# AlvinHon/ring-zk

Measured on AMD Instinct MI355X. Metric: proofs/sec (commit+challenge+response+verify), N=1024, batch=4096; NTT GB/s vs HBM peak, higher is better.
Workload: dtype u32

## Files before the change

ring_zk_amd/csrc/rzk_rowprog.h:

```cpp
#pragma once
#include "rzk_wave.h"

namespace rzk {

__device__ __forceinline__ int32_t canon_lo(int64_t c, uint32_t qhalf, uint32_t& bad) {
  bad |= (uint32_t)(((uint64_t)c + qhalf) >> 32);
  return (int32_t)c;
}
__device__ __forceinline__ int32_t canon_lo_mx(int64_t c, uint32_t qhalf, uint32_t& bad, uint32_t& mx) {
  const uint64_t s = (uint64_t)c + qhalf;
  bad |= (uint32_t)(s >> 32);
  const uint32_t lo = (uint32_t)s;
  mx = lo > mx ? lo : mx;
  return (int32_t)c;
}
__device__ __forceinline__ void canon_pair(const longlong2 t, uint32_t qhalf, uint32_t& bad, uint32_t& mx, int32_t& lo0,
                                           int32_t& lo1) {
  lo0 = canon_lo_mx(t.x, qhalf, bad, mx);
  lo1 = canon_lo_mx(t.y, qhalf, bad, mx);
}
__device__ __forceinline__ bool canon_fail(uint32_t bad, uint32_t mx, uint32_t qhalf) {
  return __any((bad != 0) | (mx > 2u * qhalf)) != 0;
}
__device__ __forceinline__ void input_fault(const Operands& ops, uint8_t* flags, uint32_t bo, int lane) {
// ... 279 lines not shown
    suma += a[i] < 0 ? 0u - ua : ua;
  }
  const double bound = (double)TM::sum_u56(suma) * (double)TM::max_u32(maxv);
  const int npass = __builtin_amdgcn_readfirstlane(bound < 4.0e18 ? 1 : 2);
  int32_t* list = ext + S::WORDS;
  uint32_t lbase = 0, ltotal = 1;
  if (LIST) {
    const uint32_t mine = shift_count_nonzeros<E>(a);
    const uint32_t w = (uint32_t)__builtin_amdgcn_readfirstlane(lane >> 6);
    if ((lane & 63) == 0) list[2 * kShiftListCap + w] = (int32_t)mine;
    TM::sync();
    const uint32_t c0 = (uint32_t)__builtin_amdgcn_readfirstlane(list[2 * kShiftListCap]);
    const uint32_t c1 = (uint32_t)__builtin_amdgcn_readfirstlane(list[2 * kShiftListCap + 1]);
    lbase = w ? c0 : 0u;
    ltotal = c0 + c1;
  }
  bool started = false;
#pragma unroll 1
  for (int pass = 0; pass < npass; ++pass) {
    if (npass == 2) {
      uint32_t u0 = 0, u1 = 0, u2 = 0;
      TM::sync();
      shift_fill_from<LOGN, PAIR, LL>(pv, lane, ext, pass == 0 ? SHIFT_LOW16 : SHIFT_HIGH16, false, false, qhalf, u0, u1, u2);
    }
    if (!LIST || npass == 2) TM::sync();
#pragma unroll 1
    for (uint32_t r0 = 0; r0 < (ltotal ? ltotal : 1u); r0 += LIST ? (uint32_t)kShiftListCap : 1u) {
      uint32_t nent = 0;
      if (LIST) {
        if (r0 || pass) TM::sync();
        shift_list_write<LOGN, PAIR, LL>(a, lane, lbase, r0, list);
        TM::sync();
        nent = ltotal - r0 < (uint32_t)kShiftListCap ? ltotal - r0 : (uint32_t)kShiftListCap;
      }
#pragma unroll 1
      for (int ch = 0; ch < NCH; ++ch) {
        int64_t acc[H];
#pragma unroll
        for (int i = 0; i < H; ++i) acc[i] = 0;
        if (LIST) shift_scan_list<LOGN, PAIR, LL, H>(acc, list, nent, lane, ext + ch * (S::LANES * H));
        else shift_scan<LOGN, PAIR, H>(acc, a, lane, ext + ch * (S::LANES * H));
#pragma unroll
        for (int i = 0; i < H; ++i) {
          uint32_t u = zq_from_i64(acc[i], T.crt);
          if (pass) u = montq_u(u, T.crt.r48q, T.crt);
          if (TO_MEM) {
            uint32_t* slot = res + S::j(lane, i) + ch * (S::LANES * H);
            const uint32_t cur = (fresh && !started) ? 0u : *slot;
            *slot = minus ? subq(cur, u, q) : addq(cur, u, q);
          } else {
#pragma unroll
            for (int c = 0; c < NCH; ++c) {
              const uint32_t cur = res[c * H + i];
              const uint32_t nw = minus ? subq(cur, u, q) : addq(cur, u, q);
              res[c * H + i] = c == ch ? nw : cur;
            }
          }
        }
      }
      started = true;
    }
  }
}

template <int LOGN>
__device__ __forceinline__ bool shift_product_bytes(uint32_t* res, bool minus, const int32_t* a, const int64_t* __restrict__ pv,
                                                    int lane, int32_t* slab, const DevTables& T, bool& fault, bool trusted) {
  using S = ShiftGeo<LOGN, true>;
  using B = ByteGeo<LOGN>;
  constexpr int E = S::E;
  const uint32_t q = T.crt.q, qhalf = T.crt.qhalf;
  uint32_t* img = reinterpret_cast<uint32_t*>(slab);
  uint32_t vbad = 0, vmx = 0, maxv = 0, suma = 0;
#pragma unroll
  for (int i = 0; i < E; ++i) {
    const uint32_t ua = (uint32_t)a[i], aa = a[i] < 0 ? 0u - ua : ua;
    suma += aa < 256u ? aa : 256u;
  }
  const uint32_t norm1 = wave_sum_u32(suma);
  if (norm1 > 255u) return false;
  wave_sync();
  constexpr int GH = S::G / 2;
  const longlong2* __restrict__ p = reinterpret_cast<const longlong2*>(pv) + lane;
#pragma unroll 1
  for (int h = 0; h < 2; ++h) {
    int32_t vh[2 * GH];
#pragma unroll
    for (int g = 0; g < GH; ++g) {
      const longlong2 t = ld_stream(p + (h * GH + g) * 64);
      if (trusted) vh[2 * g] = (int32_t)t.x, vh[2 * g + 1] = (int32_t)t.y;
      else canon_pair(t, qhalf, vbad, vmx, vh[2 * g], vh[2 * g + 1]);
    }
#pragma unroll
    for (int g = 0; g < GH; ++g) {
#pragma unroll
      for (int c = 0; c < 2; ++c) {
        const uint32_t uv = (uint32_t)vh[2 * g + c], av = vh[2 * g + c] < 0 ? 0u - uv : uv;
        maxv = av > maxv ? av : maxv;
      }
      shift_bytes_put_raw<LOGN>(vh[2 * g], vh[2 * g + 1], lane, h * GH + g, img);
    }
    if (h == 0 && wave_max_u32(maxv) > 127u) return false;
  }
  const uint32_t bias = wave_max_u32(maxv);
  if (!shift_bytes_ok(norm1, bias)) return false;
  if (!trusted) fault = fault || canon_fail(vbad, vmx, qhalf);
  wave_sync();
  shift_bytes_bias<LOGN>(lane, bias, img);
  wave_sync();
  uint32_t acc[B::W];
#pragma unroll
  for (int k = 0; k < B::W; ++k) acc[k] = 0;
#pragma unroll
  for (int i = 0; i < E; ++i) {
    uint64_t mask = __ballot(a[i] != 0);
    while (mask) {
      const int l = __builtin_ctzll(mask);
      mask &= mask - 1;
      const int32_t coef = __builtin_amdgcn_readlane(a[i], l);
      int ln = lane;
      asm volatile("" : "+v"(ln));
      shift_bytes_accum<LOGN>(acc, ln, S::off(i) + 2 * l, coef, img);
    }
  }
  wave_sync();
  shift_bytes_park<LOGN>(acc, lane, img);
  wave_sync();
  int32_t prod[E];
  shift_bytes_take<LOGN>(prod, lane, norm1 * bias, img);
#pragma unroll
  for (int i = 0; i < E; ++i) {
    const uint32_t u = zq_from_centered(prod[i], q);
    res[i] = minus ? subq(res[i], u, q) : addq(res[i], u, q);
  }
  return true;
}

template <int LOGN, class TM>
__device__ __forceinline__ void store_operand_image(const uint32_t* x, const Operands& ops, uint32_t op, uint32_t off, uint32_t b,
                                                    int pi, int lane, float nrm2, bool first) {
  using G = Geo<LOGN, TM::LL>;
  if (!ops.oimg || op != ops.oimg_op || off >= 32u) return;
  const int ci = ops.oimg_col[off];
  if (ci < 0) return;
  const size_t oslot = (size_t)b * ops.oimg_n + (uint32_t)ci;
  uint4* __restrict__ dst = reinterpret_cast<uint4*>(ops.oimg + (oslot * kKeyImages + pi) * G::N);
#pragma unroll
  for (int g = 0; g < G::E / 4; ++g) dst[G::key4(lane, g)] = make_uint4(x[4 * g], x[4 * g + 1], x[4 * g + 2], x[4 * g + 3]);
  if (lane == 0) {
    if (first) ops.oimg_l2[oslot] = (double)nrm2;
    ops.oimg_np[oslot] = (uint8_t)(pi + 1);
  }
}

template <int LOGN, bool HAS_VEC, bool OPQ = false, class TM = WaveTeam, bool DD = false>
__device__ __forceinline__ void term_direct(uint32_t* acc, const Term tm, const Operands& ops, uint32_t b,
                                            uint32_t bo, int lane, uint32_t* lds, const uint32_t* __restrict__ twf,
                                            const PrimeConsts& pc, int pi, const uint32_t* __restrict__ key_ntt,
                                            const double* __restrict__ key_l2, bool first, float& bound,
                                            uint8_t* __restrict__ flags, uint32_t qhalf) {
  using G = Geo<LOGN, TM::LL>;
  constexpr int E = G::E;
  constexpr int N = G::N;
  int ln = lane;
  RZK_OPAQUE(ln);
  uint32_t x[E];
  float nb = 0.f;
  bool below = true, fault = false;
  const bool chk = first && (tm.kind & (TERM_CHECK | TERM_CHECK2));
  const bool trusted = ops.trusted != 0;
  bool from_image = false;
  size_t oslot = 0;
  if (DD && (tm.kind & TERM_KIND_MASK) == TERM_DD && ops.oimg) {
    const uint32_t summand = tm.b_off / ops.oimg_k, col = tm.b_off - summand * ops.oimg_k;
    const int ci = col < 32u ? ops.oimg_col[col] : -1;
    if (ci >= 0) {
      oslot = ((size_t)bo * ops.oimg_group + summand) * ops.oimg_n + (uint32_t)ci;
      from_image = (int)ops.oimg_np[oslot] > pi;
    }
  }
  if (DD) from_image = __builtin_amdgcn_readfirstlane((int)from_image) != 0;
  if (DD && from_image) {
    const uint4* __restrict__ ip = reinterpret_cast<const uint4*>(ops.oimg + (oslot * kKeyImages + pi) * N);
#pragma unroll
    for (int g = 0; g < E / 4; ++g) {
      const uint4 iv = ip[G::key4(ln, g)];
      x[4 * g] = iv.x, x[4 * g + 1] = iv.y, x[4 * g + 2] = iv.z, x[4 * g + 3] = iv.w;
    }
    nb = (float)ops.oimg_l2[oslot];
  } else {
    load_lift<LOGN, TM, kRowLoadMode<TM>>(x, operand_ptr(ops, tm.b_op, tm.b_off, b, bo, N), ln, pc, first, nb, chk, ops.norm_limit, below, qhalf, trusted, fault);
    if (chk && !below && (lane & 63) == 0) fail_check(flags + bo, ops.pad != 0, (tm.kind & TERM_CHECK2) != 0);
    wave_fwd<LOGN, TM>(x, ln, lds, twf, pc);
  }
  if (HAS_VEC && (tm.kind & TERM_KIND_MASK) == TERM_VEC) {
    uint32_t xb[E];
#pragma unroll
    for (int c = 0; c < E; ++c) xb[c] = csub(mont_lazy(x[c], pc.ninv_r2, pc.p, pc.npinv), pc.p);
    float na = 0.f;
    bool unused_below = true;
    load_lift<LOGN, TM, kRowLoadMode<TM>>(x, operand_ptr(ops, tm.a_op, tm.a_off, b, bo, N), ln, pc, first, na, false, 0, unused_below, qhalf, trusted, fault);
    wave_fwd<LOGN, TM>(x, ln, lds, twf, pc);
    if (first) bound = bound_fma(na, nb, bound);
    if (tm.sign >= 0) {
#pragma unroll
      for (int c = 0; c < E; ++c) acc[c] = mac_add(acc[c], x[c], xb[c], pc);
    } else {
#pragma unroll
      for (int c = 0; c < E; ++c) acc[c] = mac_sub(acc[c], x[c], xb[c], pc);
    }
  } else {
    const bool dk = (tm.kind & TERM_KIND_MASK) == TERM_DKEY || (tm.kind & TERM_KIND_MASK) == TERM_DD;
    const size_t image = dk ? (size_t)bo * ops.dkey_n + tm.a_off : (size_t)tm.a_off;
    if (first) bound = bound_fma((float)(dk ? ops.dkey_l2[image] : key_l2[image]), nb, bound);
    const uint4* __restrict__ kp = reinterpret_cast<const uint4*>((dk ? ops.dkey_img : key_ntt) + (image * kKeyImages + pi) * N);
    if (tm.sign >= 0) {
#pragma unroll
      for (int g = 0; g < E / 4; ++g) {
        const uint4 kv = kp[G::key4(ln, g)];
        acc[4 * g + 0] = mac_add(acc[4 * g + 0], x[4 * g + 0], kv.x, pc);
        acc[4 * g + 1] = mac_add(acc[4 * g + 1], x[4 * g + 1], kv.y, pc);
        acc[4 * g + 2] = mac_add(acc[4 * g + 2], x[4 * g + 2], kv.z, pc);
        acc[4 * g + 3] = mac_add(acc[4 * g + 3], x[4 * g + 3], kv.w, pc);
      }
    } else {
#pragma unroll
      for (int g = 0; g < E / 4; ++g) {
        const uint4 kv = kp[G::key4(ln, g)];
        acc[4 * g + 0] = mac_sub(acc[4 * g + 0], x[4 * g + 0], kv.x, pc);
        acc[4 * g + 1] = mac_sub(acc[4 * g + 1], x[4 * g + 1], kv.y, pc);
        acc[4 * g + 2] = mac_sub(acc[4 * g + 2], x[4 * g + 2], kv.z, pc);
        acc[4 * g + 3] = mac_sub(acc[4 * g + 3], x[4 * g + 3], kv.w, pc);
      }
    }
  }
  if (fault) input_fault(ops, flags, bo, lane);
}

template <int LOGN, bool OPQ = false, class TM = WaveTeam>
__device__ __forceinline__ void inverse_and_fold(int pi, int np, uint32_t* acc, int lane, uint32_t* lds,
                                                 const uint32_t* __restrict__ twi, const PrimeConsts& pc,
                                                 uint32_t* st_lds, uint32_t* __restrict__ st_glb, const DevTables& T) {
  using G = Geo<LOGN, TM::LL>;
  constexpr int E = G::E;
  int li = lane;
  RZK_OPAQUE(li);
  wave_inv<LOGN, TM>(acc, li, lds, twi, pc);
  if (pi == 0) {
#pragma unroll
    for (int e = 0; e < E; ++e) st_lds[G::j_p1(li, e)] = crt_fold0(acc[e], np, T.pc, T.crt);
  } else if (pi == 1) {
    uint32_t d0[E];
#pragma unroll
    for (int e = 0; e < E; ++e) {
      d0[e] = st_lds[G::j_p1(li, e)];
      acc[e] = crt_digit1(acc[e], d0[e], np, T.pc, T.crt);
    }
    if (np == 3) {
#pragma unroll
      for (int e = 0; e < E; ++e) st_glb[G::j_p1(li, e)] = crt_value01_modp2(d0[e], acc[e], T.pc, T.crt);
    }
#pragma unroll
    for (int e = 0; e < E; ++e) st_lds[G::j_p1(li, e)] = crt_value01_modq(d0[e], acc[e], T.crt);
  } else {
#pragma unroll
    for (int e = 0; e < E; ++e) {
      uint32_t a = st_lds[G::j_p1(li, e)];
      crt_fold2(acc[e], T.pc, T.crt, a, st_glb[G::j_p1(li, e)]);
      st_lds[G::j_p1(li, e)] = a;
    }
  }
}

template <int LOGN, class TM = WaveTeam>
__device__ __forceinline__ void checked_add_verdicts(const Program* __restrict__ prog, const Row row, const Operands& ops,
                                                     uint32_t b, uint32_t bo, int lane, const float* add_ss,
                                                     uint8_t* __restrict__ flags) {
  using G = Geo<LOGN, TM::LL>;
#pragma unroll 1
  for (uint32_t a = 0; a < row.nadds && a < 4; ++a) {
    const AddTerm ad = table_load(&prog->adds[row.add0 + a]);
    if (!(ad.op & (ADD_CHECK | ADD_CHECK2))) continue;
    float part = 0.f;
#pragma unroll
    for (int sl = 0; sl < 4; ++sl) part = (sl == (int)a) ? add_ss[sl] : part;
    const double sfl = (double)TM::sum_f32(part), lim = (double)ops.norm_limit;
    bool below;
    if (sfl * (1.0 + 2.0 * (double)kNormSlack) < lim) {
      below = true;
    } else if (sfl * (1.0 - 2.0 * (double)kNormSlack) >= lim) {
      below = false;
    } else {
      const int64_t* __restrict__ src = operand_ptr(ops, ad.op & ADD_OP_MASK, ad.off, b, bo, G::N);
      int32_t v[G::E];
#pragma unroll
      for (int e = 0; e < G::E; ++e) v[e] = (int32_t)src[G::j_p1(lane, e)];
      below = TM::sum_u56(lane_sum_sq_exact<G::E>(v)) < ops.norm_limit;
    }
    if (!below && (lane & 63) == 0) fail_check(flags + bo, ops.pad != 0, (ad.op & ADD_CHECK2) != 0);
  }
}

template <int LOGN, int CH, class TM = WaveTeam>
__device__ __forceinline__ void add_chunk(uint32_t* u, const AddTerm ad, uint32_t a, const int64_t* __restrict__ src, int lane,
                                          int e0, uint32_t q, uint32_t qhalf, bool trusted, uint32_t& in_bad, uint32_t& in_mx,
                                          float* add_ss) {
  using G = Geo<LOGN, TM::LL>;
  int32_t av[CH];
  if (trusted) {
#pragma unroll
    for (int i = 0; i < CH; ++i) av[i] = (int32_t)ld_stream(src + G::j_p1(lane, e0 + i));
  } else {
#pragma unroll
    for (int i = 0; i < CH; ++i) av[i] = canon_lo_mx(ld_stream(src + G::j_p1(lane, e0 + i)), qhalf, in_bad, in_mx);
  }
  if (ad.op & (ADD_CHECK | ADD_CHECK2)) {
    float sq = 0.f;
#pragma unroll
    for (int i = 0; i < CH; ++i) {
      const float f = (float)av[i];
      sq = __builtin_fmaf(f, f, sq);
    }
    const uint32_t slot = a < 4 ? a : 3;
#pragma unroll
    for (int sl = 0; sl < 4; ++sl) add_ss[sl] += (sl == (int)slot) ? sq : 0.f;
  }
  if (ad.sign >= 0) {
#pragma unroll
    for (int i = 0; i < CH; ++i) u[i] = addq(u[i], zq_from_centered(av[i], q), q);
  } else {
#pragma unroll
    for (int i = 0; i < CH; ++i) u[i] = subq(u[i], zq_from_centered(av[i], q), q);
  }
}

template <int LOGN, class TM = WaveTeam>
__device__ __forceinline__ void row_epilogue(const Program* __restrict__ prog, const Row row, const Operands& ops,
                                             uint32_t b, uint32_t bo, int lane, bool has_terms, int np,
                                             const uint32_t* st_lds, const DevTables& T, uint8_t* __restrict__ flags,
                                             const uint32_t* __restrict__ st_sh = nullptr) {
  using G = Geo<LOGN, TM::LL>;
  constexpr int E = G::E;
  constexpr int N = G::N;
  int nz = 0;
  constexpr int CH = kEpiChunk < E ? kEpiChunk : E;
  const uint32_t q = T.crt.q;
  const bool trusted = ops.trusted != 0;
  float add_ss[4] = {0.f, 0.f, 0.f, 0.f};
  uint32_t in_bad = 0, in_mx = 0;
#pragma unroll
  for (int e0 = 0; e0 < E; e0 += CH) {
    uint32_t u[CH];
    if (has_terms) {
#pragma unroll
      for (int i = 0; i < CH; ++i) u[i] = crt_finish_zq(st_lds[G::j_p1(lane, e0 + i)], np, T.crt);
    } else {
#pragma unroll
      for (int i = 0; i < CH; ++i) u[i] = 0;
    }
    if (st_sh) {
#pragma unroll
      for (int i = 0; i < CH; ++i) u[i] = addq(u[i], st_sh[G::j_p1(lane, e0 + i)], q);
    }
#pragma unroll 1
    for (uint32_t a = 0; a < row.nadds; ++a) {
      const AddTerm ad = table_load(&prog->adds[row.add0 + a]);
      add_chunk<LOGN, CH, TM>(u, ad, a, operand_ptr(ops, ad.op & ADD_OP_MASK, ad.off, b, bo, N), lane, e0, q, T.crt.qhalf, trusted,
                          in_bad, in_mx, add_ss);
    }
    if (row.mode == MODE_STORE) {
      int64_t* __restrict__ dst = const_cast<int64_t*>(operand_ptr(ops, row.out_op, row.out_off, b, bo, N));
#pragma unroll
      for (int i = 0; i < CH; ++i) st_stream(dst + G::j_p1(lane, e0 + i), center_from_zq(u[i], T.crt));
    } else {
#pragma unroll
      for (int i = 0; i < CH; ++i) nz |= (u[i] != 0);
    }
  }
  if (row.mode != MODE_STORE) {
    if (__any(nz) && (lane & 63) == 0) flags[bo] = 0;
  }
  if (row.nadds && !trusted && canon_fail(in_bad, in_mx, T.crt.qhalf)) input_fault(ops, flags, bo, lane);
  if (ops.norm_limit) checked_add_verdicts<LOGN, TM>(prog, row, ops, b, bo, lane, add_ss, flags);
}

__device__ __forceinline__ int primes_for(float fbound, const DevTables& T) {
  const double bound = (double)fbound * (1.0 + 0x1p-12);
  const int np = bound <= T.cap[1] ? 1 : (bound <= T.cap[2] ? 2 : 3);
  return __builtin_amdgcn_readfirstlane(np);
}

}
```

ring_zk_amd/csrc/rzk_unit.h:

```cpp
#pragma once
#include "rzk_rowprog.h"

namespace rzk {

constexpr int kScratchLines = 6;
#ifndef RZK_STAMPS
#define RZK_STAMPS 0
#endif
#if RZK_STAMPS
#define RZK_T0() const uint64_t t_sec0 = __builtin_amdgcn_s_memtime()
#define RZK_T1(acc) acc += __builtin_amdgcn_s_memtime() - t_sec0
#else
#define RZK_T0() do { } while (0)
#define RZK_T1(acc) do { } while (0)
#endif

__device__ __forceinline__ void set_priority_level(uint32_t level) {
  if (level == 0) __builtin_amdgcn_s_setprio(3);
  else if (level == 1) __builtin_amdgcn_s_setprio(2);
  else if (level == 2) __builtin_amdgcn_s_setprio(1);
  else __builtin_amdgcn_s_setprio(0);
}
__device__ __forceinline__ void set_progress_priority(uint32_t done, uint32_t total) {
  set_priority_level(__builtin_amdgcn_readfirstlane(total ? (done * 4u) / total : 0u));
}
template <int LOGN, bool to_regs, bool MINUS, class TM = WaveTeam>
__device__ __forceinline__ void mac_park_signed(uint32_t* x, const uint32_t* mul, uint4* P4, int lane, bool init,
                                                const PrimeConsts& pc) {
  using G = Geo<LOGN, TM::LL>;
  constexpr int E = G::E;
  if (init && !MINUS) {
#pragma unroll
    for (int g = 0; g < E / 4; ++g) {
      uint32_t as[4];
#pragma unroll
      for (int i = 0; i < 4; ++i) as[i] = mont_lazy(x[4 * g + i], mul[4 * g + i], pc.p, pc.npinv);
      if (to_regs) {
#pragma unroll
        for (int i = 0; i < 4; ++i) x[4 * g + i] = as[i];
      } else {
        P4[G::own4(lane, g)] = make_uint4(as[0], as[1], as[2], as[3]);
      }
    }
    return;
  }
#pragma unroll
  for (int g = 0; g < E / 4; ++g) {
    uint4 a = make_uint4(0, 0, 0, 0);
    if (!init) a = P4[G::own4(lane, g)];
    uint32_t as[4] = {a.x, a.y, a.z, a.w};
#pragma unroll
    for (int i = 0; i < 4; ++i)
      as[i] = MINUS ? mac_sub(as[i], x[4 * g + i], mul[4 * g + i], pc) : mac_add(as[i], x[4 * g + i], mul[4 * g + i], pc);
    if (to_regs) {
#pragma unroll
      for (int i = 0; i < 4; ++i) x[4 * g + i] = as[i];
    } else {
      P4[G::own4(lane, g)] = make_uint4(as[0], as[1], as[2], as[3]);
    }
  }
}
template <int LOGN, bool to_regs, class TM = WaveTeam>
__device__ __forceinline__ void mac_park(uint32_t* x, const uint32_t* mul, bool minus, uint4* P4, int lane, bool init,
                                         const PrimeConsts& pc) {
  if (minus) mac_park_signed<LOGN, to_regs, true, TM>(x, mul, P4, lane, init, pc);
  else mac_park_signed<LOGN, to_regs, false, TM>(x, mul, P4, lane, init, pc);
}

template <int LOGN, bool OPQ, class TM = WaveTeam>
__device__ __forceinline__ bool inverse_fold_global(int pi, int np, uint32_t* acc, int lane, uint32_t* lds,
                                                    const uint32_t* __restrict__ twi, const PrimeConsts& pc,
                                                    uint32_t* __restrict__ stA, uint32_t* __restrict__ stB,
                                                    const DevTables& T) {
  using G = Geo<LOGN, TM::LL>;
  constexpr int E = G::E;
  int li = lane;
  RZK_OPAQUE(li);
  uint4* __restrict__ A4 = reinterpret_cast<uint4*>(stA);
  uint4* __restrict__ B4 = reinterpret_cast<uint4*>(stB);
  constexpr bool EARLY = E <= 16;
  uint4 sa[E / 4], sb[E / 4];
  if (EARLY && pi >= 1) {
#pragma unroll
    for (int g = 0; g < E / 4; ++g) sa[g] = A4[G::own4(li, g)];
  }
  if (EARLY && pi == 2) {
#pragma unroll
    for (int g = 0; g < E / 4; ++g) sb[g] = B4[G::own4(li, g)];
  }
  wave_inv<LOGN, TM>(acc, li, lds, twi, pc);
  if (!EARLY && pi >= 1) {
#pragma unroll
    for (int g = 0; g < E / 4; ++g) sa[g] = A4[G::own4(li, g)];
  }
  if (!EARLY && pi == 2) {
#pragma unroll
    for (int g = 0; g < E / 4; ++g) sb[g] = B4[G::own4(li, g)];
  }
  if (pi == 0) {
    if (np == 1) {
#pragma unroll
      for (int e = 0; e < E; ++e) acc[e] = crt1_zq(acc[e], T.pc, T.crt);
      return true;
    }
    if (np == 2) {
#pragma unroll
      for (int e = 0; e < E; ++e) acc[e] = crt2_digit0(acc[e], T.pc);
    } else {
#pragma unroll
      for (int e = 0; e < E; ++e) acc[e] = crt_fold0(acc[e], np, T.pc, T.crt);
    }
#pragma unroll
    for (int g = 0; g < E / 4; ++g) A4[G::own4(li, g)] = make_uint4(acc[4 * g], acc[4 * g + 1], acc[4 * g + 2], acc[4 * g + 3]);
    return false;
  }
  if (pi == 1 && np == 2) {
#pragma unroll
    for (int g = 0; g < E / 4; ++g) {
      const uint4 dv = sa[g];
      const uint32_t d0[4] = {dv.x, dv.y, dv.z, dv.w};
#pragma unroll
      for (int i = 0; i < 4; ++i) acc[4 * g + i] = crt2_zq(acc[4 * g + i], d0[i], T.pc, T.crt);
    }
    return true;
  }
  if (pi == 1) {
#pragma unroll
    for (int g = 0; g < E / 4; ++g) {
      const uint4 dv = sa[g];
      const uint32_t d0[4] = {dv.x, dv.y, dv.z, dv.w};
      uint32_t va[4], vb[4];
#pragma unroll
      for (int i = 0; i < 4; ++i) {
        const uint32_t d1 = crt_digit1(acc[4 * g + i], d0[i], np, T.pc, T.crt);
        va[i] = crt_value01_modq(d0[i], d1, T.crt);
        vb[i] = crt_value01_modp2(d0[i], d1, T.pc, T.crt);
      }
      A4[G::own4(li, g)] = make_uint4(va[0], va[1], va[2], va[3]);
      B4[G::own4(li, g)] = make_uint4(vb[0], vb[1], vb[2], vb[3]);
    }
    return false;
  }
#pragma unroll
  for (int g = 0; g < E / 4; ++g) {
    const uint4 av = sa[g], bv = sb[g];
    uint32_t a[4] = {av.x, av.y, av.z, av.w};
    const uint32_t bb[4] = {bv.x, bv.y, bv.z, bv.w};
#pragma unroll
    for (int i = 0; i < 4; ++i) {
      crt_fold2(acc[4 * g + i], T.pc, T.crt, a[i], bb[i]);
      acc[4 * g + i] = crt_finish_zq(a[i], 3, T.crt);
    }
  }
  return true;
}

template <int LOGN, int CHMAX = 16, class TM = WaveTeam>
__device__ __forceinline__ void finish_row(uint32_t* u, const Program* __restrict__ prog, const Row row,
                                           const Operands& ops, uint32_t b, uint32_t bo, int lane, const DevTables& T,
                                           uint8_t* __restrict__ flags, const uint32_t* __restrict__ st_sh) {
  using G = Geo<LOGN, TM::LL>;
  constexpr int E = G::E;
  constexpr int N = G::N;
  const uint32_t q = T.crt.q, qhalf = T.crt.qhalf;
  const bool trusted = ops.trusted != 0;
  if (st_sh) {
#pragma unroll
    for (int e = 0; e < E; ++e) u[e] = addq(u[e], st_sh[G::j_p1(lane, e)], q);
  }
  constexpr int CH = E < CHMAX ? E : CHMAX;
  float add_ss[4] = {0.f, 0.f, 0.f, 0.f};
  uint32_t in_bad = 0, in_mx = 0;
  int nz = 0;
#pragma unroll
  for (int e0 = 0; e0 < E; e0 += CH) {
#pragma unroll 1
    for (uint32_t a = 0; a < row.nadds; ++a) {
      const AddTerm ad = table_load(&prog->adds[row.add0 + a]);
      add_chunk<LOGN, CH, TM>(u + e0, ad, a, operand_ptr(ops, ad.op & ADD_OP_MASK, ad.off, b, bo, N), lane, e0, q, qhalf, trusted,
                          in_bad, in_mx, add_ss);
    }
    if (row.mode == MODE_STORE) {
      int64_t* __restrict__ dst = const_cast<int64_t*>(operand_ptr(ops, row.out_op, row.out_off, b, bo, N));
#pragma unroll
      for (int i = 0; i < CH; ++i) st_stream(dst + G::j_p1(lane, e0 + i), center_from_zq(u[e0 + i], T.crt));
    } else {
#pragma unroll
      for (int i = 0; i < CH; ++i) nz |= (u[e0 + i] != 0);
    }
  }
  if (row.mode != MODE_STORE) {
    if (__any(nz) && (lane & 63) == 0) flags[bo] = 0;
  }
  if (row.nadds && !trusted && canon_fail(in_bad, in_mx, qhalf)) input_fault(ops, flags, bo, lane);
  if (ops.norm_limit) checked_add_verdicts<LOGN, TM>(prog, row, ops, b, bo, lane, add_ss, flags);
}

template <int LOGN, bool HAS_VEC, bool HAS_SHIFT, class TM = WaveTeam>
__global__ void __launch_bounds__(TM::kTeamsPerBlock << TM::LL, ((LOGN <= 10 && HAS_VEC) || TM::LL == 7 ? 4 : 1))
unit_kernel(const Program* __restrict__ prog, const WaveProgram* __restrict__ wp, const Operands ops,
            const uint32_t* __restrict__ key_ntt, const double* __restrict__ key_l2, const DevTables* __restrict__ Tp,
            const uint32_t* __restrict__ tw_all, uint32_t* __restrict__ scratch, uint8_t* __restrict__ flags,
            const uint32_t ntasks, const uint32_t units_per_task, const uint32_t tasks_per_entry,
            const uint32_t work_per_task) {
  using G = Geo<LOGN, TM::LL>;
  constexpr int E = G::E;
  constexpr int N = G::N;
  constexpr bool OPQ = true;
  extern __shared__ __attribute__((aligned(16))) uint32_t smem[];
  const int lane = threadIdx.x & (G::LANES - 1);
  const uint32_t wave = __builtin_amdgcn_readfirstlane(threadIdx.x >> TM::LL);
  constexpr int WPB = TM::kTeamsPerBlock;
  uint32_t* lds = smem + wave * (G::LDS_WORDS + N);
  uint4* P4 = reinterpret_cast<uint4*>(lds + G::LDS_WORDS);
  uint32_t* st = scratch + ((size_t)blockIdx.x * WPB + wave) * (size_t)(kScratchLines * N + 16);
  uint32_t* st_sh = st + 4 * N;
#if RZK_STAMPS
  const uint64_t stamp0 = __builtin_amdgcn_s_memrealtime();
  const uint64_t cyc0 = __builtin_amdgcn_s_memtime();
  uint64_t t_load = 0, t_fwd = 0, t_mac = 0, t_inv = 0, t_fin = 0, t_rot = 0;
#endif
  const DevTables& T = *Tp;
  const uint32_t qhalf = T.crt.qhalf;
  const bool trusted = ops.trusted != 0;
  const uint32_t nunits = wp->nunits;

  const uint32_t first_task = blockIdx.x * WPB + wave;
  const uint32_t my_tasks = first_task < ntasks ? (ntasks - first_task + gridDim.x * WPB - 1) / (gridDim.x * WPB) : 0;
  const uint32_t work_total = my_tasks * work_per_task;
  uint32_t work_done = 0;
#define RZK_STEP_PRIORITY()                             \
  do {                                                  \
    set_progress_priority(work_done, work_total);       \
    ++work_done;                                        \
  } while (0)

  for (uint32_t task = first_task; task < ntasks; task += gridDim.x * WPB) {
    const uint32_t b = task / tasks_per_entry;
    const uint32_t u0 = (task - b * tasks_per_entry) * units_per_task;
    const uint32_t u1 = u0 + units_per_task < nunits ? u0 + units_per_task : nunits;
    const uint32_t bo = ops.group > 1 ? b / ops.group : b;
    if (ops.preset) {
      if (lane == 0) flags[bo] = (uint8_t)ops.preset;
      if (TM::LL != 6) TM::sync();
    }
#pragma unroll 1
    for (uint32_t ui = u0; ui < u1; ++ui) {
      const Unit un = table_load(&wp->units[ui]);
      const Row rowA = table_load(&prog->rows[un.rowA]);
      const bool pair = un.rowB != kNoRow;
      const uint32_t un_items = un.nitems;
      const bool null_unit = un_items == 0;
      const bool has_shift = HAS_SHIFT && rowA.nshift > 0;
      if (has_shift) {
        bool fault = false;
        RZK_T0();
#pragma unroll 1
        for (uint32_t t = 0; t < rowA.nshift; ++t) {
          const Term tm = table_load(&prog->terms[rowA.term0 + rowA.nterms + t]);
          const int64_t* __restrict__ pa = operand_ptr(ops, tm.a_op, tm.a_off, b, bo, N);
          int32_t a[E];
          if (trusted) {
#pragma unroll
            for (int e = 0; e < E; ++e) a[e] = (int32_t)pa[G::j_p1(lane, e)];
          } else {
            uint32_t abad = 0, amx = 0;
#pragma unroll
            for (int e = 0; e < E; ++e) a[e] = canon_lo_mx(pa[G::j_p1(lane, e)], qhalf, abad, amx);
            fault = fault || canon_fail(abad, amx, qhalf);
          }
          shift_product<LOGN, false, true, TM>(st_sh, t == 0, tm.sign < 0, a, operand_ptr(ops, tm.b_op, tm.b_off, b, bo, N), lane,
                                           reinterpret_cast<int32_t*>(lds), T, fault, trusted);
        }
        if (fault) input_fault(ops, flags, bo, lane);
        TM::sync();
        RZK_T1(t_rot);
      }
      int np = null_unit ? 1 : kMaxPrimes;
      const uint32_t nit = null_unit ? 1u : un_items;
      float boundA = 0.f, boundB = 0.f;
#pragma unroll 1
      for (int pi = 0; pi < np; ++pi) {
        const PrimeConsts pc = T.pc[pi];
        const uint32_t* __restrict__ twf = tw_all + (size_t)(2 * pi) * kTableLen;
        const bool first = pi == 0;
        bool fault = false;
#pragma unroll 1
        for (uint32_t it = 0; it < nit; ++it) {
          const bool last = it + 1 == nit;
          RZK_STEP_PRIORITY();
          int ln = lane;
          RZK_OPAQUE(ln);
          uint32_t acc[E];
#pragma unroll
          for (int c = 0; c < E; ++c) acc[c] = 0;
          if (!null_unit) {
            const Item im = table_load(&wp->items[un.item0 + it]);
            uint32_t x[E];
            float nb = 0.f;
            bool below = true;
            const bool chk = first && (im.flags & (TERM_CHECK | TERM_CHECK2));
            {
              RZK_T0();
              load_lift<LOGN, TM>(x, operand_ptr(ops, im.b_op, im.b_off, b, bo, N), ln, pc, first, nb, chk, ops.norm_limit, below, qhalf,
                              trusted, fault);
              RZK_T1(t_load);
            }
            if (chk && !below && (lane & 63) == 0) fail_check(flags + bo, ops.pad != 0, (im.flags & TERM_CHECK2) != 0);
            const bool vec = HAS_VEC && im.kind == ITEM_VEC;
            constexpr bool EARLY = E <= 16 && !HAS_VEC;
            uint32_t kreg[E];
            const uint4* __restrict__ kpA = reinterpret_cast<const uint4*>(key_ntt + ((size_t)im.keyA * kKeyImages + pi) * N);
            if (EARLY && !vec && im.keyA != kNoKey) {
#pragma unroll
              for (int g = 0; g < E / 4; ++g) {
                const uint4 kv = kpA[G::key4(ln, g)];
                kreg[4 * g] = kv.x, kreg[4 * g + 1] = kv.y, kreg[4 * g + 2] = kv.z, kreg[4 * g + 3] = kv.w;
              }
            }
            {
              RZK_T0();
              wave_fwd<LOGN, TM>(x, ln, lds, twf, pc);
              RZK_T1(t_fwd);
            }
            if (!EARLY && !vec && im.keyA != kNoKey) {
#pragma unroll
              for (int g = 0; g < E / 4; ++g) {
                const uint4 kv = kpA[G::key4(ln, g)];
                kreg[4 * g] = kv.x, kreg[4 * g + 1] = kv.y, kreg[4 * g + 2] = kv.z, kreg[4 * g + 3] = kv.w;
              }
            }
            uint32_t xb[E];
            if (vec) {
#pragma unroll
              for (int c = 0; c < E; ++c) xb[c] = csub(mont_lazy(x[c], pc.ninv_r2, pc.p, pc.npinv), pc.p);
              float na = 0.f;
              bool unused_below = true;
              load_lift<LOGN, TM>(x, operand_ptr(ops, im.a_op, im.a_off, b, bo, N), ln, pc, first, na, false, 0, unused_below, qhalf,
                              trusted, fault);
              wave_fwd<LOGN, TM>(x, ln, lds, twf, pc);
              if (first) boundA = bound_fma(na, nb, boundA);
            } else if (first) {
              if (im.keyA != kNoKey) boundA = bound_fma((float)key_l2[im.keyA], nb, boundA);
              if (pair && im.keyB != kNoKey) boundB = bound_fma((float)key_l2[im.keyB], nb, boundB);
            }
            const bool feedsA = vec || im.keyA != kNoKey;
            if (!last) {
              RZK_T0();
              if (vec) mac_park<LOGN, false, TM>(x, xb, im.signA < 0, P4, ln, it == 0, pc);
              else if (feedsA) mac_park<LOGN, false, TM>(x, kreg, im.signA < 0, P4, ln, it == 0, pc);
              RZK_T1(t_mac);
              continue;
            }
            RZK_T0();
            if (fault) input_fault(ops, flags, bo, lane);
            if (first) np = primes_for(boundA > boundB ? boundA : boundB, T);
#pragma unroll
            for (int c = 0; c < E; ++c) acc[c] = x[c];
            if (vec) {
              mac_park<LOGN, true, TM>(acc, xb, im.signA < 0, P4, ln, it == 0, pc);
            } else if (feedsA) {
              mac_park<LOGN, true, TM>(acc, kreg, im.signA < 0, P4, ln, it == 0, pc);
            } else {
#pragma unroll
              for (int g = 0; g < E / 4; ++g) {
                const uint4 v = P4[G::own4(ln, g)];
                acc[4 * g] = v.x, acc[4 * g + 1] = v.y, acc[4 * g + 2] = v.z, acc[4 * g + 3] = v.w;
              }
            }
            if (pair) {
              const uint4* __restrict__ kb = reinterpret_cast<const uint4*>(key_ntt + ((size_t)im.keyB * kKeyImages + pi) * N);
              uint32_t kbr[E];
#pragma unroll
              for (int g = 0; g < E / 4; ++g) {
                const uint4 kv = kb[G::key4(ln, g)];
                kbr[4 * g] = kv.x, kbr[4 * g + 1] = kv.y, kbr[4 * g + 2] = kv.z, kbr[4 * g + 3] = kv.w;
              }
              mac_park<LOGN, false, TM>(x, kbr, im.signB < 0, P4, ln, true, pc);
            }
            RZK_T1(t_mac);
          }
#pragma unroll 1
          for (uint32_t r = 0; r < (pair ? 2u : 1u); ++r) {
            if (r == 1) {
#pragma unroll
              for (int g = 0; g < E / 4; ++g) {
                const uint4 v = P4[G::own4(ln, g)];
                acc[4 * g] = v.x, acc[4 * g + 1] = v.y, acc[4 * g + 2] = v.z, acc[4 * g + 3] = v.w;
              }
            }
            bool done = true;
            RZK_STEP_PRIORITY();
            if (!null_unit) {
              RZK_T0();
              done = inverse_fold_global<LOGN, OPQ, TM>(pi, np, acc, lane, lds, twf + kTableLen, pc, st + (size_t)(2 * r) * N,
                                                    st + (size_t)(2 * r + 1) * N, T);
              RZK_T1(t_inv);
            }
            if (done) {
              RZK_T0();
              finish_row<LOGN, 16, TM>(acc, prog, table_load(&prog->rows[r ? un.rowB : un.rowA]), ops, b, bo, lane, T, flags,
                               (has_shift && r == 0) ? st_sh : nullptr);
              RZK_T1(t_fin);
            }
          }
        }
      }
    }
  }
#undef RZK_STEP_PRIORITY
#if RZK_STAMPS
  if (lane == 0) {
    const uint64_t stamp1 = __builtin_amdgcn_s_memrealtime();
    uint32_t hwid;
    asm volatile("s_getreg_b32 %0, hwreg(HW_REG_HW_ID)" : "=s"(hwid));
    uint32_t xcc;
    asm volatile("s_getreg_b32 %0, hwreg(HW_REG_XCC_ID)" : "=s"(xcc));
    uint32_t* o = st + kScratchLines * N;
    o[0] = (uint32_t)stamp0, o[1] = (uint32_t)(stamp0 >> 32), o[2] = (uint32_t)stamp1, o[3] = (uint32_t)(stamp1 >> 32);
    o[4] = hwid, o[5] = xcc, o[6] = blockIdx.x, o[7] = wave;
    const uint64_t cyc1 = __builtin_amdgcn_s_memtime();
    o[8] = (uint32_t)(cyc1 - cyc0);
    o[9] = (uint32_t)t_load, o[10] = (uint32_t)t_fwd, o[11] = (uint32_t)t_mac, o[12] = (uint32_t)t_inv, o[13] = (uint32_t)t_fin, o[14] = (uint32_t)t_rot;
  }
#endif
}

template <int LOGN, class TM = WaveTeam>
__device__ __forceinline__ void load_measure(int32_t* v, const int64_t* __restrict__ src, int lane, bool measure, float& nrm2,
                                             bool check, uint64_t limit, bool& below, uint32_t qhalf, bool trusted, bool& fault) {
  using G = Geo<LOGN, TM::LL>;
  if (!measure || trusted) {
#pragma unroll
    for (int e = 0; e < G::E; ++e) v[e] = (int32_t)src[G::j_p1(lane, e)];
  } else {
    uint32_t bad = 0, mx = 0;
#pragma unroll
    for (int e = 0; e < G::E; ++e) v[e] = canon_lo_mx(src[G::j_p1(lane, e)], qhalf, bad, mx);
    fault = fault || canon_fail(bad, mx, qhalf);
  }
  if (measure) {
    const float ss = TM::sum_f32(lane_sum_sq_f32<G::E>(v));
    nrm2 = norm2_upper(ss);
    if (check) below = norm_below<G::E, TM>(v, ss, limit);
  }
}
template <int LOGN, class TM, class P4T>
__device__ __forceinline__ void unpark(uint32_t* a, P4T P4, int lane) {
  using G = Geo<LOGN, TM::LL>;
#pragma unroll
  for (int g = 0; g < G::E / 4; ++g) {
    const uint4 v = P4[G::own4(lane, g)];
    a[4 * g] = v.x, a[4 * g + 1] = v.y, a[4 * g + 2] = v.z, a[4 * g + 3] = v.w;
  }
}

template <int LOGN, int LL>
struct IoCfg {
  static constexpr bool P1_FULL = LOGN == 9;
  static constexpr bool B0_LDS = LOGN == 9;
  static constexpr int N = 1 << LOGN;
  static constexpr int SLAB = Geo<LOGN, LL>::LDS_WORDS;
  static constexpr int OFF_P1 = SLAB + N;
  static constexpr int OFF_B0 = OFF_P1 + (P1_FULL ? N : 0);
  static constexpr int WORDS = OFF_B0 + (B0_LDS ? N : 0);
};
template <int LOGN, bool HAS_SHIFT, class TM = WaveTeam>
__global__ void __launch_bounds__(TM::kTeamsPerBlock << TM::LL, (TM::LL == 7 || LOGN == 10 ? 4 : 1))
unit_io_kernel(const Program* __restrict__ prog, const WaveProgram* __restrict__ wp, const Operands ops,
               const uint32_t* __restrict__ key_ntt, const double* __restrict__ key_l2, const DevTables* __restrict__ Tp,
               const uint32_t* __restrict__ tw_all, uint32_t* __restrict__ scratch, uint8_t* __restrict__ flags,
               const uint32_t ntasks, const uint32_t units_per_task, const uint32_t tasks_per_entry,
               const uint32_t work_per_task) {
  using G = Geo<LOGN, TM::LL>;
  constexpr int E = G::E;
  constexpr int N = G::N;
  constexpr bool OPQ = true;
  extern __shared__ __attribute__((aligned(16))) uint32_t smem[];
  const int lane = threadIdx.x & (G::LANES - 1);
  const uint32_t wave = __builtin_amdgcn_readfirstlane(threadIdx.x >> TM::LL);
  constexpr int TPB = TM::kTeamsPerBlock;
  using IO = IoCfg<LOGN, TM::LL>;
  constexpr bool P1L = IO::P1_FULL, B0L = IO::B0_LDS;
  uint32_t* lds = smem + wave * IO::WORDS;
  uint4* P4 = reinterpret_cast<uint4*>(lds + IO::SLAB);
  uint4* P41 = reinterpret_cast<uint4*>(lds + IO::OFF_P1);
  uint4* PB0 = reinterpret_cast<uint4*>(lds + IO::OFF_B0);
  uint32_t* st = scratch + ((size_t)blockIdx.x * TPB + wave) * (size_t)(kScratchLines * N + 16);
  uint32_t* st_sh = st + 4 * N;
#if RZK_STAMPS
  const uint64_t stamp0 = __builtin_amdgcn_s_memrealtime();
  const uint64_t cyc0 = __builtin_amdgcn_s_memtime();
#endif
  const DevTables& T = *Tp;
  const uint32_t qhalf = T.crt.qhalf;
  const bool trusted = ops.trusted != 0;
  const uint32_t nunits = wp->nunits;
  const uint32_t first_task = blockIdx.x * TPB + wave;
  const uint32_t my_tasks = first_task < ntasks ? (ntasks - first_task + gridDim.x * TPB - 1) / (gridDim.x * TPB) : 0;
  const uint32_t work_total = my_tasks * work_per_task;
  uint32_t work_done = 0;
#define RZK_STEP_PRIORITY()                             \
  do {                                                  \
    set_progress_priority(work_done, work_total);       \
    ++work_done;                                        \
  } while (0)

  for (uint32_t task = first_task; task < ntasks; task += gridDim.x * TPB) {
    const uint32_t b = task / tasks_per_entry;
    const uint32_t u0 = (task - b * tasks_per_entry) * units_per_task;
    const uint32_t u1 = u0 + units_per_task < nunits ? u0 + units_per_task : nunits;
    const uint32_t bo = ops.group > 1 ? b / ops.group : b;
    if (ops.preset) {
      if (lane == 0) flags[bo] = (uint8_t)ops.preset;
      if (TM::LL != 6) TM::sync();
    }
#pragma unroll 1
    for (uint32_t ui = u0; ui < u1; ++ui) {
      const Unit un = table_load(&wp->units[ui]);
      const Row rowA = table_load(&prog->rows[un.rowA]);
      const bool pair = un.rowB != kNoRow;
      const uint32_t nit = un.nitems;
      const bool has_shift = HAS_SHIFT && rowA.nshift > 0;
      if (has_shift) {
        bool fault = false;
#pragma unroll 1
        for (uint32_t t = 0; t < rowA.nshift; ++t) {
          const Term tm = table_load(&prog->terms[rowA.term0 + rowA.nterms + t]);
          const int64_t* __restrict__ pa = operand_ptr(ops, tm.a_op, tm.a_off, b, bo, N);
          int32_t a[E];
          if (trusted) {
#pragma unroll
            for (int e = 0; e < E; ++e) a[e] = (int32_t)pa[G::j_p1(lane, e)];
          } else {
            uint32_t abad = 0, amx = 0;
#pragma unroll
            for (int e = 0; e < E; ++e) a[e] = canon_lo_mx(pa[G::j_p1(lane, e)], qhalf, abad, amx);
            fault = fault || canon_fail(abad, amx, qhalf);
          }
          shift_product<LOGN, false, true, TM>(st_sh, t == 0, tm.sign < 0, a, operand_ptr(ops, tm.b_op, tm.b_off, b, bo, N), lane,
                                           reinterpret_cast<int32_t*>(lds), T, fault, trusted);
        }
        if (fault) input_fault(ops, flags, bo, lane);
        TM::sync();
      }
      if (nit == 0) {
        uint32_t u[E];
#pragma unroll
        for (int e = 0; e < E; ++e) u[e] = 0;
        RZK_STEP_PRIORITY();
        finish_row<LOGN, 16, TM>(u, prog, rowA, ops, b, bo, lane, T, flags, has_shift ? st_sh : nullptr);
        continue;
      }
      float boundA = 0.f, boundB = 0.f;
      bool fault = false, haveA = false;
      int np = 2;
#pragma unroll 1
      for (int pass = 0; pass < (np == 3 ? 2 : 1); ++pass) {
        haveA = false;
#pragma unroll 1
        for (uint32_t it = 0; it < nit; ++it) {
          const bool last = it + 1 == nit;
          int ln = lane;
          RZK_OPAQUE(ln);
          const Item im = table_load(&wp->items[un.item0 + it]);
          const int64_t* __restrict__ src = operand_ptr(ops, im.b_op, im.b_off, b, bo, N);
          const bool chk = pass == 0 && (im.flags & (TERM_CHECK | TERM_CHECK2));
          const bool feedsA = im.keyA != kNoKey;
          const bool feedsB = pair && last && im.keyB != kNoKey;
          const int pi0 = pass == 0 ? 0 : 2, pi1 = pass == 0 ? 2 : 3;
          constexpr bool RETAIN = E <= 8;
          int32_t vkeep[RETAIN ? E : 1];
          if (RETAIN) {
            float nb = 0.f;
            bool below = true;
            load_measure<LOGN, TM>(vkeep, src, ln, pass == 0, nb, chk, ops.norm_limit, below, qhalf, trusted, fault);
            if (chk && !below && (lane & 63) == 0) fail_check(flags + bo, ops.pad != 0, (im.flags & TERM_CHECK2) != 0);
            if (pass == 0) {
              if (feedsA) boundA = bound_fma((float)key_l2[im.keyA], nb, boundA);
              if (pair && im.keyB != kNoKey) boundB = bound_fma((float)key_l2[im.keyB], nb, boundB);
            }
          }
#pragma unroll 1
          for (int pi = pi0; pi < pi1; ++pi) {
            RZK_STEP_PRIORITY();
            RZK_OPAQUE(ln);
            const PrimeConsts pc = T.pc[pi];
            const uint32_t* __restrict__ twf = tw_all + (size_t)(2 * pi) * kTableLen;
            uint32_t x[E];
            if (RETAIN) {
#pragma unroll
              for (int e = 0; e < E; ++e) x[e] = lift(vkeep[RETAIN ? e : 0], pc);
            } else if (pi == pi0) {
              int32_t v[E];
              float nb = 0.f;
              bool below = true;
              load_measure<LOGN, TM>(v, src, ln, pass == 0, nb, chk, ops.norm_limit, below, qhalf, trusted, fault);
              if (chk && !below && (lane & 63) == 0) fail_check(flags + bo, ops.pad != 0, (im.flags & TERM_CHECK2) != 0);
              if (pass == 0) {
                if (feedsA) boundA = bound_fma((float)key_l2[im.keyA], nb, boundA);
                if (pair && im.keyB != kNoKey) boundB = bound_fma((float)key_l2[im.keyB], nb, boundB);
              }
#pragma unroll
              for (int e = 0; e < E; ++e) x[e] = lift(v[e], pc);
            } else {
              const int32_t* __restrict__ lo32 = reinterpret_cast<const int32_t*>(src);
#pragma unroll
              for (int e = 0; e < E; ++e) x[e] = lift(lo32[2 * G::j_p1(ln, e)], pc);
            }
            constexpr bool EARLY = false;
            const uint4* __restrict__ kpA = reinterpret_cast<const uint4*>(key_ntt + ((size_t)(feedsA ? im.keyA : 0) * kKeyImages + pi) * N);
            uint32_t kreg[E];
            if (EARLY && feedsA) {
              int lk = ln;
              asm volatile("" : "+v"(lk) : "v"(x[E - 1]));
#pragma unroll
              for (int g = 0; g < E / 4; ++g) {
                const uint4 kv = kpA[G::key4(lk, g)];
                kreg[4 * g] = kv.x, kreg[4 * g + 1] = kv.y, kreg[4 * g + 2] = kv.z, kreg[4 * g + 3] = kv.w;
              }
            }
            wave_fwd<LOGN, TM>(x, ln, lds, twf, pc);
            if (feedsA) {
              if (!EARLY) {
#pragma unroll
                for (int g = 0; g < E / 4; ++g) {
                  const uint4 kv = kpA[G::key4(ln, g)];
                  kreg[4 * g] = kv.x, kreg[4 * g + 1] = kv.y, kreg[4 * g + 2] = kv.z, kreg[4 * g + 3] = kv.w;
                }
              }
              if (pi == 0) mac_park<LOGN, false, TM>(x, kreg, im.signA < 0, P4, ln, !haveA, pc);
              else if (P1L && pi == 1) mac_park<LOGN, false, TM>(x, kreg, im.signA < 0, P41, ln, !haveA, pc);
              else mac_park<LOGN, false, TM>(x, kreg, im.signA < 0, reinterpret_cast<uint4*>(st + (pi == 1 ? 0 : 3) * N), ln, !haveA, pc);
            }
            if (feedsB) {
              const uint4* __restrict__ kpB = reinterpret_cast<const uint4*>(key_ntt + ((size_t)im.keyB * kKeyImages + pi) * N);
              uint32_t kbr[E];
              int lb = ln;
              asm volatile("" : "+v"(lb));
#pragma unroll
              for (int g = 0; g < E / 4; ++g) {
                const uint4 kv = kpB[G::key4(lb, g)];
                kbr[4 * g] = kv.x, kbr[4 * g + 1] = kv.y, kbr[4 * g + 2] = kv.z, kbr[4 * g + 3] = kv.w;
              }
              if (B0L && pi == 0) mac_park<LOGN, false, TM>(x, kbr, im.signB < 0, PB0, ln, true, pc);
              else mac_park<LOGN, false, TM>(x, kbr, im.signB < 0, reinterpret_cast<uint4*>(st + (pi == 0 ? 1 : (pi == 1 ? 2 : 5)) * N), ln, true, pc);
            }
          }
          haveA = haveA || feedsA;
        }
        if (pass == 0) {
          if (fault) input_fault(ops, flags, bo, lane);
          np = primes_for(boundA > boundB ? boundA : boundB, T);
          np = np < 2 ? 2 : np;
        }
      }
#pragma unroll 1
      for (uint32_t r = 0; r < (pair ? 2u : 1u); ++r) {
        int li = lane;
        RZK_OPAQUE(li);
        const bool have = r == 1 || haveA;
        uint32_t u[E];
        if (!have) {
#pragma unroll
          for (int e = 0; e < E; ++e) u[e] = 0;
        } else {
          uint32_t a[E];
          if (r == 0) unpark<LOGN, TM>(a, const_cast<const uint4*>(P4), li);
          else if (B0L) unpark<LOGN, TM>(a, const_cast<const uint4*>(PB0), li);
          else unpark<LOGN, TM>(a, reinterpret_cast<const uint4*>(st + 1 * N), li);
          RZK_STEP_PRIORITY();
          RZK_OPAQUE(li);
          wave_inv<LOGN, TM>(a, li, lds, tw_all + (size_t)(2 * 0 + 1) * kTableLen, T.pc[0]);
          if (np == 2) {
#pragma unroll
            for (int e = 0; e < E; ++e) u[e] = crt2_digit0(a[e], T.pc);
            if (P1L && r == 0) unpark<LOGN, TM>(a, const_cast<const uint4*>(P41), li);
            else unpark<LOGN, TM>(a, reinterpret_cast<const uint4*>(st + (r == 0 ? 0 : 2) * N), li);
            RZK_STEP_PRIORITY();
            RZK_OPAQUE(li);
            wave_inv<LOGN, TM>(a, li, lds, tw_all + (size_t)(2 * 1 + 1) * kTableLen, T.pc[1]);
#pragma unroll
            for (int e = 0; e < E; ++e) u[e] = crt2_zq(a[e], u[e], T.pc, T.crt);
          } else {
            uint32_t wb[E];
#pragma unroll
            for (int e = 0; e < E; ++e) u[e] = crt_fold0(a[e], 3, T.pc, T.crt);
            if (P1L && r == 0) unpark<LOGN, TM>(a, const_cast<const uint4*>(P41), li);
            else unpark<LOGN, TM>(a, reinterpret_cast<const uint4*>(st + (r == 0 ? 0 : 2) * N), li);
            RZK_STEP_PRIORITY();
            RZK_OPAQUE(li);
            wave_inv<LOGN, TM>(a, li, lds, tw_all + (size_t)(2 * 1 + 1) * kTableLen, T.pc[1]);
#pragma unroll
            for (int e = 0; e < E; ++e) {
              wb[e] = 0;
              crt_fold1(a[e], 3, T.pc, T.crt, u[e], wb[e]);
            }
            unpark<LOGN, TM>(a, reinterpret_cast<const uint4*>(st + (r == 0 ? 3 : 5) * N), li);
            RZK_STEP_PRIORITY();
            RZK_OPAQUE(li);
            wave_inv<LOGN, TM>(a, li, lds, tw_all + (size_t)(2 * 2 + 1) * kTableLen, T.pc[2]);
#pragma unroll
            for (int e = 0; e < E; ++e) {
              crt_fold2(a[e], T.pc, T.crt, u[e], wb[e]);
              u[e] = crt_finish_zq(u[e], 3, T.crt);
// ... 28 lines not shown
```

Measured before the change: 15.57 million.

## Prefetch first add-term operand during inverse NTT to hide load latency

```diff
diff --git a/ring_zk_amd/csrc/rzk_rowprog.h b/ring_zk_amd/csrc/rzk_rowprog.h
--- a/ring_zk_amd/csrc/rzk_rowprog.h
+++ b/ring_zk_amd/csrc/rzk_rowprog.h
@@ -605,36 +605,48 @@
 }
 
 template <int LOGN, int CH, class TM = WaveTeam>
+__device__ __forceinline__ void add_request(int64_t* raw, const int64_t* __restrict__ src, int lane, int e0) {
+  using G = Geo<LOGN, TM::LL>;
+#pragma unroll
+  for (int i = 0; i < CH; ++i) raw[i] = ld_stream(src + G::j_p1(lane, e0 + i));
+}
+template <int CH>
+__device__ __forceinline__ void add_apply(uint32_t* u, const AddTerm ad, uint32_t a, const int64_t* raw, uint32_t q, uint32_t qhalf,
+                                          bool trusted, uint32_t& in_bad, uint32_t& in_mx, float* add_ss) {
+  int32_t av[CH];
+  if (trusted) {
+#pragma unroll
+    for (int i = 0; i < CH; ++i) av[i] = (int32_t)raw[i];
+  } else {
+#pragma unroll
+    for (int i = 0; i < CH; ++i) av[i] = canon_lo_mx(raw[i], qhalf, in_bad, in_mx);
+  }
+  if (ad.op & (ADD_CHECK | ADD_CHECK2)) {
+    float sq = 0.f;
+#pragma unroll
+    for (int i = 0; i < CH; ++i) {
+      const float f = (float)av[i];
+      sq = __builtin_fmaf(f, f, sq);
+    }
+    const uint32_t slot = a < 4 ? a : 3;
+#pragma unroll
+    for (int sl = 0; sl < 4; ++sl) add_ss[sl] += (sl == (int)slot) ? sq : 0.f;
+  }
+  if (ad.sign >= 0) {
+#pragma unroll
+    for (int i = 0; i < CH; ++i) u[i] = addq(u[i], zq_from_centered(av[i], q), q);
+  } else {
+#pragma unroll
+    for (int i = 0; i < CH; ++i) u[i] = subq(u[i], zq_from_centered(av[i], q), q);
+  }
+}
+template <int LOGN, int CH, class TM = WaveTeam>
 __device__ __forceinline__ void add_chunk(uint32_t* u, const AddTerm ad, uint32_t a, const int64_t* __restrict__ src, int lane,
                                           int e0, uint32_t q, uint32_t qhalf, bool trusted, uint32_t& in_bad, uint32_t& in_mx,
                                           float* add_ss) {
-  using G = Geo<LOGN, TM::LL>;
-  int32_t av[CH];
-  if (trusted) {
-#pragma unroll
-    for (int i = 0; i < CH; ++i) av[i] = (int32_t)ld_stream(src + G::j_p1(lane, e0 + i));
-  } else {
-#pragma unroll
-    for (int i = 0; i < CH; ++i) av[i] = canon_lo_mx(ld_stream(src + G::j_p1(lane, e0 + i)), qhalf, in_bad, in_mx);
-  }
-  if (ad.op & (ADD_CHECK | ADD_CHECK2)) {
-    float sq = 0.f;
-#pragma unroll
-    for (int i = 0; i < CH; ++i) {
-      const float f = (float)av[i];
-      sq = __builtin_fmaf(f, f, sq);
-    }
-    const uint32_t slot = a < 4 ? a : 3;
-#pragma unroll
-    for (int sl = 0; sl < 4; ++sl) add_ss[sl] += (sl == (int)slot) ? sq : 0.f;
-  }
-  if (ad.sign >= 0) {
-#pragma unroll
-    for (int i = 0; i < CH; ++i) u[i] = addq(u[i], zq_from_centered(av[i], q), q);
-  } else {
-#pragma unroll
-    for (int i = 0; i < CH; ++i) u[i] = subq(u[i], zq_from_centered(av[i], q), q);
-  }
+  int64_t raw[CH];
+  add_request<LOGN, CH, TM>(raw, src, lane, e0);
+  add_apply<CH>(u, ad, a, raw, q, qhalf, trusted, in_bad, in_mx, add_ss);
 }
 
 template <int LOGN, class TM = WaveTeam>
diff --git a/ring_zk_amd/csrc/rzk_unit.h b/ring_zk_amd/csrc/rzk_unit.h
--- a/ring_zk_amd/csrc/rzk_unit.h
+++ b/ring_zk_amd/csrc/rzk_unit.h
@@ -4,6 +4,14 @@
 namespace rzk {
 
 constexpr int kScratchLines = 6;
+#ifndef RZK_LOAD_AHEAD
+#define RZK_LOAD_AHEAD 1
+#endif
+template <int K, class Tp>
+__device__ __forceinline__ void any_value(Tp* v) {
+#pragma unroll
+  for (int i = 0; i < K; ++i) asm volatile("" : "=v"(v[i]));
+}
 #ifndef RZK_STAMPS
 #define RZK_STAMPS 0
 #endif
@@ -67,11 +75,12 @@
   else mac_park_signed<LOGN, to_regs, false, TM>(x, mul, P4, lane, init, pc);
 }
 
-template <int LOGN, bool OPQ, class TM = WaveTeam>
+
+template <int LOGN, bool OPQ, class TM = WaveTeam, class AheadFn>
 __device__ __forceinline__ bool inverse_fold_global(int pi, int np, uint32_t* acc, int lane, uint32_t* lds,
                                                     const uint32_t* __restrict__ twi, const PrimeConsts& pc,
                                                     uint32_t* __restrict__ stA, uint32_t* __restrict__ stB,
-                                                    const DevTables& T) {
+                                                    const DevTables& T, AheadFn request_ahead) {
   using G = Geo<LOGN, TM::LL>;
   constexpr int E = G::E;
   int li = lane;
@@ -97,6 +106,7 @@
 #pragma unroll
     for (int g = 0; g < E / 4; ++g) sb[g] = B4[G::own4(li, g)];
   }
+  request_ahead(li);
   if (pi == 0) {
     if (np == 1) {
 #pragma unroll
@@ -155,27 +165,38 @@
   return true;
 }
 
-template <int LOGN, int CHMAX = 16, class TM = WaveTeam>
+template <int LOGN, int CHMAX = 16, class TM = WaveTeam, bool AHEAD = false>
 __device__ __forceinline__ void finish_row(uint32_t* u, const Program* __restrict__ prog, const Row row,
                                            const Operands& ops, uint32_t b, uint32_t bo, int lane, const DevTables& T,
-                                           uint8_t* __restrict__ flags, const uint32_t* __restrict__ st_sh) {
+                                           uint8_t* __restrict__ flags, const uint32_t* __restrict__ st_sh,
+                                           bool ahead = false, const AddTerm ahead_ad = AddTerm(), const int64_t* ahead_raw = nullptr) {
   using G = Geo<LOGN, TM::LL>;
   constexpr int E = G::E;
   constexpr int N = G::N;
   const uint32_t q = T.crt.q, qhalf = T.crt.qhalf;
   const bool trusted = ops.trusted != 0;
-  if (st_sh) {
-#pragma unroll
-    for (int e = 0; e < E; ++e) u[e] = addq(u[e], st_sh[G::j_p1(lane, e)], q);
-  }
-  constexpr int CH = E < CHMAX ? E : CHMAX;
   float add_ss[4] = {0.f, 0.f, 0.f, 0.f};
   uint32_t in_bad = 0, in_mx = 0;
+  auto add_rotations = [&]() {
+    if (st_sh) {
+#pragma unroll
+      for (int e = 0; e < E; ++e) u[e] = addq(u[e], st_sh[G::j_p1(lane, e)], q);
+    }
+  };
+  add_rotations();
+  uint32_t a_done = 0;
+  if constexpr (AHEAD) {
+    if (ahead) {
+      add_apply<E>(u, ahead_ad, 0, ahead_raw, q, qhalf, trusted, in_bad, in_mx, add_ss);
+      a_done = 1;
+    }
+  }
+  constexpr int CH = E < CHMAX ? E : CHMAX;
   int nz = 0;
 #pragma unroll
   for (int e0 = 0; e0 < E; e0 += CH) {
 #pragma unroll 1
-    for (uint32_t a = 0; a < row.nadds; ++a) {
+    for (uint32_t a = a_done; a < row.nadds; ++a) {
       const AddTerm ad = table_load(&prog->adds[row.add0 + a]);
       add_chunk<LOGN, CH, TM>(u + e0, ad, a, operand_ptr(ops, ad.op & ADD_OP_MASK, ad.off, b, bo, N), lane, e0, q, qhalf, trusted,
                           in_bad, in_mx, add_ss);
@@ -197,7 +218,7 @@
 }
 
 template <int LOGN, bool HAS_VEC, bool HAS_SHIFT, class TM = WaveTeam>
-__global__ void __launch_bounds__(TM::kTeamsPerBlock << TM::LL, ((LOGN <= 10 && HAS_VEC) || TM::LL == 7 ? 4 : 1))
+__global__ void __launch_bounds__(TM::kTeamsPerBlock << TM::LL, ((LOGN <= 10 && (HAS_VEC || RZK_LOAD_AHEAD)) || TM::LL == 7 ? 4 : 1))
 unit_kernel(const Program* __restrict__ prog, const WaveProgram* __restrict__ wp, const Operands ops,
             const uint32_t* __restrict__ key_ntt, const double* __restrict__ key_l2, const DevTables* __restrict__ Tp,
             const uint32_t* __restrict__ tw_all, uint32_t* __restrict__ scratch, uint8_t* __restrict__ flags,
@@ -207,6 +228,7 @@
   constexpr int E = G::E;
   constexpr int N = G::N;
   constexpr bool OPQ = true;
+  constexpr bool AHEAD = RZK_LOAD_AHEAD && E <= 16 && !HAS_VEC && TM::LL == 6;
   extern __shared__ __attribute__((aligned(16))) uint32_t smem[];
   const int lane = threadIdx.x & (G::LANES - 1);
   const uint32_t wave = __builtin_amdgcn_readfirstlane(threadIdx.x >> TM::LL);
@@ -317,6 +339,8 @@
                 const uint4 kv = kpA[G::key4(ln, g)];
                 kreg[4 * g] = kv.x, kreg[4 * g + 1] = kv.y, kreg[4 * g + 2] = kv.z, kreg[4 * g + 3] = kv.w;
               }
+            } else if (EARLY && AHEAD) {
+              any_value<E>(kreg);
             }
             {
               RZK_T0();
@@ -391,16 +415,36 @@
             }
             bool done = true;
             RZK_STEP_PRIORITY();
+            bool ahead = false;
+            AddTerm ahead_ad = AddTerm();
+            int64_t ahead_raw[AHEAD ? E : 1];
             if (!null_unit) {
               RZK_T0();
+              auto request_ahead = [&](int li) __attribute__((always_inline)) {
+                if constexpr (AHEAD) {
+                  if (pi + 1 == np && pi < 2) {
+                    const Row rw = table_load(&prog->rows[r ? un.rowB : un.rowA]);
+                    if (rw.nadds) {
+                      ahead = true;
+                      ahead_ad = table_load(&prog->adds[rw.add0]);
+                      __builtin_amdgcn_sched_barrier(0);
+                      add_request<LOGN, E, TM>(ahead_raw, operand_ptr(ops, ahead_ad.op & ADD_OP_MASK, ahead_ad.off, b, bo, N), li, 0);
+                      __builtin_amdgcn_sched_barrier(0);
+                    }
+                  }
+                  if (!ahead) any_value<E>(ahead_raw);
+                }
+              };
               done = inverse_fold_global<LOGN, OPQ, TM>(pi, np, acc, lane, lds, twf + kTableLen, pc, st + (size_t)(2 * r) * N,
-                                                    st + (size_t)(2 * r + 1) * N, T);
+                                                    st + (size_t)(2 * r + 1) * N, T, request_ahead);
               RZK_T1(t_inv);
+            } else if constexpr (AHEAD) {
+              any_value<E>(ahead_raw);
             }
             if (done) {
               RZK_T0();
-              finish_row<LOGN, 16, TM>(acc, prog, table_load(&prog->rows[r ? un.rowB : un.rowA]), ops, b, bo, lane, T, flags,
-                               (has_shift && r == 0) ? st_sh : nullptr);
+              finish_row<LOGN, 16, TM, AHEAD>(acc, prog, table_load(&prog->rows[r ? un.rowB : un.rowA]), ops, b, bo, lane, T, flags,
+                                      (has_shift && r == 0) ? st_sh : nullptr, ahead, ahead_ad, ahead_raw);
               RZK_T1(t_fin);
             }
           }
```

Measured after the change: 14.63 million. -6.0%, worse.
